# samiazirar/mvtracker

Hardware: AMD Instinct MI355X
Metric: query-points*frames/sec, 4-view 24-frame 512x512 @1024 queries (higher is better)
Workload: dtype bf16; 1 GPU; c3: 4-view synthetic 24-frame 512x512, 1024 queries, bf16 (configs[2], the metric's config); 4-view 24-frame 512x512, 1024 queries per GPU, corr K=16 x 4 levels, iters=4, 3 windows, random-init weights (seeded recipe); queries_total=1024, parallelism=query-shard x1, frame_store=bf16 rows

## Files before the change

include/mvtracker_hip.h:

```cpp
#ifndef MVTRACKER_HIP_H
#define MVTRACKER_HIP_H

#include <stdint.h>

#ifdef __cplusplus
extern "C" {
#endif

#define MVT_OK 0
#define MVT_ERR_ARG 1
#define MVT_ERR_HIP_BASE 1000

#define MVT_ACT_NONE 0
#define MVT_ACT_RELU 1
#define MVT_ACT_GELU_TANH 2
#define MVT_ACT_GELU_ERF 3

int mvt_abi_version(void);
const char* mvt_build_arch(void);

int mvt_gemm(const float* A, int lda, const float* Wt, int ldw, const float* bias, const float* R, int ldr,
             float* C, int ldc, int M, int N, int K, int act, void* stream);

int mvt_conv2d(const float* in, const float* wt, const float* bias, float* out, int n, int H, int W, int Cin,
// ... 2 lines not shown
int mvt_split_bf16(const float* src, unsigned short* hi, unsigned short* lo, long long n, void* stream);
int mvt_gemm_bf16(const float* A, int lda, const unsigned short* w_hi, const unsigned short* w_lo, int ldw,
                  const float* bias, const float* R, int ldr, void* C, int ldc, int M, int N, int K, int act,
                  int io_flags , void* stream);
#define MVT_IO_IN_BF16 1
#define MVT_IO_OUT_BF16 2
#define MVT_IO_SHORT_WG 4
int mvt_conv2d_stat_slots(int H, int W, int Cin, int KH, int KW, int stride, int pad, int split );
int mvt_conv3x3s2_down_bf16(const void* in, const unsigned short* w3, const float* b3, const unsigned short* wd, const float* bd,
                            void* out3, void* outd, int n, int H, int W, int Cin, int Cout, int ldo, float* part3, float* partd,
                            void* stream);
int mvt_conv2d_bf16(const void* in, const unsigned short* wt_hi, const unsigned short* wt_lo, const float* bias,
                    void* out, int n, int H, int W, int Cin, int Cout, int KH, int KW, int stride, int pad, int ldo,
                    int act, int io_flags, const float* in_stats, float* out_partial, void* stream);
int mvt_instnorm_finish_slots(const float* partial, int slots, float* mean_rstd, int n, long long HW, int C, void* stream);

int mvt_ln_gemm_bf16(const float* A, int lda, const float* ln_w, const float* ln_b, float ln_eps,
                     const unsigned short* w_hi, const unsigned short* w_lo, int ldw, const float* bias, const float* R,
                     int ldr, float* C, int ldc, int M, int N, int K, int act, void* stream);

int mvt_mlp_fused_bf16(float* x, int ldx, const unsigned short* w1, int ldw1, const float* b1,
                       const unsigned short* w2, int ldw2, const float* b2, long long M, int C, int H, float eps,
                       void* stream);

int mvt_pack_frag_bf16(const unsigned short* w, int ld, int N, int K, unsigned short* out, void* stream);
typedef struct mvt_block_next {
  const unsigned short* w;
  const float* b;
  const float* lnw;
  const float* lnb;
// ... 389 lines not shown
```

mvtracker_amd/csrc/conv_rows.hip:

```cpp
#include <stdlib.h>

#include "common.h"

namespace {

typedef __bf16 bf16x8 __attribute__((ext_vector_type(8)));
typedef __bf16 bf16x4 __attribute__((ext_vector_type(4)));
typedef unsigned u32x4 __attribute__((ext_vector_type(4)));
typedef unsigned u32x2 __attribute__((ext_vector_type(2)));
typedef float f32x2 __attribute__((ext_vector_type(2)));
typedef short s16x2 __attribute__((ext_vector_type(2)));
typedef __bf16 bf16x2 __attribute__((ext_vector_type(2)));

#ifdef MVT_STAMPS
#ifndef MVT_STAMP_WG
#define MVT_STAMP_WG 2000
#endif
__device__ unsigned long long mvt_conv_stamp_buf[2 * 8 * 128];
#define CSTAMP(i)                                                                                                  \
  do {                                                                                                             \
    __builtin_amdgcn_sched_barrier(0);                                                                             \
    unsigned long long t_;                                                                                         \
    asm volatile("s_memtime %0\n\ts_waitcnt lgkmcnt(0)" : "=s"(t_)::"memory");                                     \
    __builtin_amdgcn_sched_barrier(0);                                                                             \
// ... 918 lines not shown
}
#endif

static int rows_nw8() {
  static const int v = getenv("MVT_ROWS_NW8") ? atoi(getenv("MVT_ROWS_NW8")) : 0;
  return v;
}
__attribute__((visibility("hidden"))) int mvt_detail_conv_rows_tile_rows(int ksize, int stride, int Ho) {
  if (ksize == 3 && stride == 1) return (rows_nw8() == 1 && Ho % 16 == 0) ? 16 : (rows_nw8() == 2 ? 4 : 8);
  if (ksize == 3) return 4;
  if (ksize == 7) return TR;
  return 8;
}
__attribute__((visibility("hidden"))) int mvt_detail_conv_rows_slots(int Ho, int Wo, int tile_rows) {
  return (int)(mvt_cdiv(Ho, tile_rows) * mvt_cdiv(Wo, TC));
}

__attribute__((visibility("hidden"))) int mvt_detail_conv_rows(const void* in, const unsigned short* w, int ldw, const float* bias, void* out,
                                                               int n, int H, int W, int Cin, int Cout, int ksize, int stride, int ldo,
                                                               int io_flags, const float* in_stats, float* out_partial,
                                                               hipStream_t stream) {
  MVT_REQUIRE((ksize == 1 || ksize == 3) && (stride == 1 || stride == 2));
  MVT_REQUIRE((!in_stats || Cin <= MAXC) && Cin % CK == 0 && (long long)H * W * Cin < (1LL << 31) && (long long)Cout * ldw < (1LL << 31));
  MVT_REQUIRE((long long)(TC + 8) * ldo * 4 < (1LL << 31));
  const int pad = ksize == 3 ? 1 : 0;
  const int Ho = (H + 2 * pad - ksize) / stride + 1, Wo = (W + 2 * pad - ksize) / stride + 1;
  RowsArgs a{};
  a.in = (const float*)in; a.w = w; a.bias = bias; a.out = (float*)out; a.in_stats = in_stats; a.out_part = out_partial;
  a.H = H; a.W = W; a.Cin = Cin; a.Cout = Cout; a.ldw = ldw; a.ldo = ldo;
  a.slots = mvt_detail_conv_rows_slots(Ho, Wo, mvt_detail_conv_rows_tile_rows(ksize, stride, Ho));
// ... 13 lines not shown
    const long long tiles = (long long)n * mvt_cdiv(Ho, NW_ * TM_) * mvt_cdiv(Wo, TC) * mvt_cdiv(Cout, bn);                        \
    MVT_REQUIRE(tiles < (1LL << 31));                                                                                              \
    const dim3 grid((unsigned)tiles);                                                                                              \
    if (n96) {                                                                                                                     \
      if (a.in_bf16) LAUNCH2(TM_, 3, KS_, S_, NW_, true);                                                                          \
      else LAUNCH2(TM_, 3, KS_, S_, NW_, false);                                                                                   \
    } else {                                                                                                                       \
      if (a.in_bf16) LAUNCH2(TM_, 2, KS_, S_, NW_, true);                                                                          \
      else LAUNCH2(TM_, 2, KS_, S_, NW_, false);                                                                                   \
    }                                                                                                                              \
  } while (0)
  const int nw8 = rows_nw8();
  if (ksize == 3 && stride == 1 && !in_stats && !(io_flags & MVT_IO_SHORT_WG) && a.in_bf16 && st_ok && Cout % BG_BN == 0 && ((uintptr_t)in & 15) == 0 && Cin % 8 == 0 &&
      ldw % 8 == 0 && ((uintptr_t)w & 15) == 0 && (long long)Cout * ldw * 2 < (1LL << 31) && (long long)H * W * Cin * 2 < (1LL << 31)) {
    const char* e = getenv("MVT_CONV_BIG");
    if (!e || atoi(e) != 0) {
      const long long tiles = (long long)n * mvt_cdiv(Ho, TR) * mvt_cdiv(Wo, TC) * (Cout / BG_BN);
      MVT_REQUIRE(tiles < (1LL << 31));
      hipLaunchKernelGGL(conv3x3_big_bf16, dim3((unsigned)tiles), dim3(512), 0, stream, a);
      return mvt_launch_status();
    }
  }
  if (ksize == 3 && stride == 1 && nw8 == 1 && Ho % 16 == 0) LAUNCH(2, 3, 1, 8);
  else if (ksize == 3 && stride == 1 && nw8 == 2) LAUNCH(1, 3, 1, 4);
  else if (ksize == 3 && stride == 1) LAUNCH(2, 3, 1, 4);
  else if (ksize == 3) LAUNCH(1, 3, 2, 4);
  else if (stride == 1) LAUNCH(2, 1, 1, 4);
  else LAUNCH(2, 1, 2, 4);
#undef LAUNCH2
#undef LAUNCH
  return mvt_launch_status();
}
// ... 62 lines not shown
```

mvtracker_amd/csrc/encoder.hip:

```cpp
#include <stdlib.h>

#include "common.h"

namespace {

template <typename TIN>
__global__ void rgb_to_nhwc4_kernel(const TIN* __restrict__ rgbs, float* __restrict__ out, int V, int T, int H, int W,
                                    long long img0, long long nimg) {
  const long long hw = (long long)H * W;
  const long long total = nimg * hw;
  for (long long i = blockIdx.x * (long long)blockDim.x + threadIdx.x; i < total; i += (long long)gridDim.x * blockDim.x) {
    long long img = i / hw;
    long long pix = i - img * hw;
    int tt = (int)((img0 + img) / V), v = (int)((img0 + img) - (long long)tt * V);
    const TIN* src = rgbs + (((long long)v * T + tt) * 3) * hw + pix;
    f32x4 o;
    o[0] = 2.0f * ((float)src[0] / 255.0f) - 1.0f;
    o[1] = 2.0f * ((float)src[hw] / 255.0f) - 1.0f;
    o[2] = 2.0f * ((float)src[2 * hw] / 255.0f) - 1.0f;
    o[3] = 0.0f;
    *reinterpret_cast<f32x4*>(out + i * 4) = o;
  }
}

// ... 65 lines not shown
  double s = 0, ss = 0;
  for (int slab = 0; slab < MVT_IN_SLABS; ++slab) {
    const double* p = partial + ((img * MVT_IN_SLABS + slab) * C + c) * 2;
    s += p[0];
    ss += p[1];
  }
  double mean = s / (double)HW;
  double var = ss / (double)HW - mean * mean;
  if (var < 0) var = 0;
  mean_rstd[i * 2] = (float)mean;
  mean_rstd[i * 2 + 1] = (float)(1.0 / sqrt(var + 1e-5));
}

constexpr int FC = 8, FL = 1024 / FC;
__global__ __launch_bounds__(1024) void instnorm_finish_slots_kernel(const float* __restrict__ partial, int slots,
                                                                     float* __restrict__ mean_rstd, long long HW, int C) {
  __shared__ double red[1024 * 2];
  const int t = threadIdx.x, c = blockIdx.x * FC + (t % FC), l = t / FC;
  const long long img = blockIdx.y;
  double s = 0, ss = 0;
  if (c < C) {
    for (int sl = l; sl < slots; sl += FL) {
      const float2 v = *reinterpret_cast<const float2*>(partial + ((img * slots + sl) * C + c) * 2);
      s += (double)v.x;
      ss += (double)v.y;
    }
  }
  red[t * 2] = s;
  red[t * 2 + 1] = ss;
  __syncthreads();
  for (int w = FL / 2; w >= 1; w >>= 1) {
    if (l < w) {
      red[t * 2] += red[(t + w * FC) * 2];
      red[t * 2 + 1] += red[(t + w * FC) * 2 + 1];
// ... 326 lines not shown
                                  int io_flags, void* stream) {
  MVT_REQUIRE((io_flags & ~MVT_IO_IN_BF16) == 0);
  MVT_REQUIRE(x && partial && mean_rstd && n > 0 && HW > 0 && C > 0 && C % 4 == 0 && C <= 256 && ldx >= C && ldx % 4 == 0);
  MVT_REQUIRE(256 % (C / 4) == 0 || C / 4 <= 64);
  hipLaunchKernelGGL(instnorm_partial_kernel, dim3(MVT_IN_SLABS, n), dim3(256), 0, mvt_stream(stream), (const float*)x, ldx, partial,
                     HW, C, io_flags & MVT_IO_IN_BF16 ? 1 : 0);
  long long total = (long long)n * C;
  hipLaunchKernelGGL(instnorm_finish_kernel, dim3((unsigned)mvt_cdiv(total, 256)), dim3(256), 0, mvt_stream(stream), partial,
                     mean_rstd, HW, C, total);
  return mvt_launch_status();
}

extern "C" int mvt_instnorm_finish_slots(const float* partial, int slots, float* mean_rstd, int n, long long HW, int C, void* stream) {
  MVT_REQUIRE(partial && mean_rstd && slots > 0 && n > 0 && HW > 0 && C > 0);
  hipLaunchKernelGGL(instnorm_finish_slots_kernel, dim3((unsigned)mvt_cdiv(C, FC), (unsigned)n), dim3(1024), 0, mvt_stream(stream),
                     partial, slots, mean_rstd, HW, C);
  return mvt_launch_status();
}

extern "C" int mvt_instnorm_apply(const void* x, const float* mean_rstd, const void* skip, const float* skip_stats, void* y,
                                  int n, long long HW, int C, int io_flags, void* stream) {
  MVT_REQUIRE(x && mean_rstd && y && n > 0 && HW > 0 && C > 0 && C % 4 == 0);
  const int both = MVT_IO_IN_BF16 | MVT_IO_OUT_BF16;
  const int skip_relu = io_flags & MVT_APPLY_SKIP_RELU ? 1 : 0;
  io_flags &= ~MVT_APPLY_SKIP_RELU;
  MVT_REQUIRE(io_flags == 0 || io_flags == both);
  MVT_REQUIRE(!skip_relu || skip_stats);
  MVT_REQUIRE(skip || !skip_stats);
  static const bool generic = getenv("MVT_APPLY_GENERIC") != nullptr;
  if (io_flags && C % 8 == 0 && C <= 2048 && HW < (1LL << 31) && !generic && ((uintptr_t)x % 16 == 0) && ((uintptr_t)y % 16 == 0) &&
      ((uintptr_t)skip % 16 == 0)) {
// ... 34 lines not shown
```

mvtracker_amd/csrc/encoder_forward.hip:

```cpp
#include "common.h"
#include <stdlib.h>

namespace {

inline long long align256(long long b) { return (b + 255) & ~255LL; }

struct Plan {
  long long stem, z0, y, s[4], d, cat, c2, part, st, total;
  long long st_ch;
};

inline Plan plan(long long n, int H, int W, int C) {
  const long long h2 = H / 2, w2 = W / 2, hs = H / 4, ws = W / 4;
  Plan P{};
  long long o = 0;
  auto take = [&](long long bytes) { const long long at = o; o += align256(bytes); return at; };
  const long long big = n * h2 * w2 * 64 * 2;
  P.stem = take(big);
  P.z0 = take(big);
  P.y = take(big);
  const int couts[4] = {64, 96, 128, 128};
  long long hh = h2, ww = w2;
  for (int l = 0; l < 4; ++l) {
    if (l) {
// ... 6 lines not shown
  P.cat = take(n * hs * ws * 416 * 2);
  P.c2 = take(n * hs * ws * 2 * C * 2);
  const long long slots_max = ((h2 + 7) / 8) * ((w2 + 31) / 32);
  P.st_ch = 2 * C > 256 ? 2 * C : 256;
  P.part = take(n * slots_max * P.st_ch * 2 * 4);
  P.st = take(8 * n * P.st_ch * 2 * 4);
  P.total = o;
  return P;
}

constexpr long long GROUP_BUDGET_SHARED = 80LL << 20;
inline int group_size(int n, int h2, int w2, int shared, int* g_out) {
  long long g = shared ? GROUP_BUDGET_SHARED / (3LL * h2 * w2 * 64 * 2) : n;
  if (g < 1) g = n;
  if (const char* e = getenv("MVT_ENC_GROUP")) {
    const long v = strtol(e, nullptr, 10);
    if (v < 0) return MVT_ERR_ARG;
    if (v > 0) g = v;
  }
  *g_out = (int)(g > n ? n : g);
  return MVT_OK;
}

}

extern "C" long long mvt_encoder_workspace_bytes(int n, int H, int W, int C) {
  if (n <= 0 || H < 16 || W < 16 || C <= 0) return -1;
  return plan(n, H, W, C).total;
}

// ... 34 lines not shown

  auto conv = [&](int ci, const void* in, int io_in, void* out, int hh, int ww, int cin, int cout, int k, int stride, int pad, int ld_out,
                  const float* in_stats, float** st_out, int io_out) -> int {
    const mvt_conv_weights& cw = w->conv[ci];
    const int ho = (hh + 2 * pad - k) / stride + 1, wo = (ww + 2 * pad - k) / stride + 1;
    const long long in_img = (long long)hh * ww * cin * (io_in & MVT_IO_IN_BF16 ? 2 : 4);
    const long long out_img = (long long)ho * wo * ld_out * (io_out & MVT_IO_OUT_BF16 ? 2 : 4);
    float* pp = nullptr;
    int slots = 0;
    if (st_out) {
      slots = mvt_conv2d_stat_slots(hh, ww, cin, k, k, stride, pad, 0);
      MVT_REQUIRE(slots > 0);
      pp = part + (long long)ga * slots * cout * 2;
    }
    ENC_TRY(mvt_conv2d_bf16(img(in, in_img), cw.w, nullptr, cw.b, img(out, out_img), gn, hh, ww, cin, cout, k, k, stride, pad, ld_out,
                            MVT_ACT_NONE, io_in | io_out | (w->short_workgroups ? MVT_IO_SHORT_WG : 0), rows_of(in_stats, cin), pp, stream));
    if (st_out) {
      *st_out = new_st();
      ENC_TRY(mvt_instnorm_finish_slots(pp, slots, (float*)rows_of(*st_out, cout), gn, (long long)ho * wo, cout, stream));
    }
    return MVT_OK;
  };

  auto stem = [&](float** st_stem) -> int {
    if (x4) return conv(0, x4, 0, base + P.stem, H, W, 4, 64, 7, 2, 3, 64, nullptr, st_stem, MVT_IO_OUT_BF16);
    const mvt_conv_weights& cw = w->conv[0];
    const int slots = mvt_detail_conv_rows_slots(h2, w2, mvt_detail_conv_rows_tile_rows(7, 2, h2));
    float* pp = part + (long long)ga * slots * 64 * 2;
    ENC_TRY(mvt_detail_stem7x7_rows_src(nullptr, rgb, rgb_u8, rgb_V, rgb_T, img0 + ga, cw.w, (7 * 32 + 63) & ~63, cw.b,
                                        img(base + P.stem, (long long)h2 * w2 * 64 * 2), gn, H, W, 64, 64, MVT_IO_OUT_BF16, pp, mvt_stream(stream)));
    *st_stem = new_st();
// ... 3 lines not shown
  auto res_block = [&](int c1, int c2, int cd, const void* xin, const float* x_stats, int hh, int ww, int cin, int cout, int stride,
                       void* zout) -> int {
    const int ho = (hh + 2 - 3) / stride + 1, wo = (ww + 2 - 3) / stride + 1;
    const long long in_img = (long long)hh * ww * cin * 2, out_img = (long long)ho * wo * cout * 2;
    float *s1 = nullptr, *s2 = nullptr, *sd = nullptr;
    static const bool no_fold = getenv("MVT_FOLD_DOWNSAMPLE") && atoi(getenv("MVT_FOLD_DOWNSAMPLE")) == 0;
    const bool fold = cd >= 0 && stride == 2 && !x_stats && cout % 32 == 0 && !no_fold;
    if (fold) {
      const int slots = mvt_conv2d_stat_slots(hh, ww, cin, 3, 3, 2, 1, 0);
      MVT_REQUIRE(slots > 0);
      float* part_3 = part + (long long)ga * slots * cout * 2;
      float* part_d = part_3 + (long long)n * slots * cout * 2;
      ENC_TRY(mvt_conv3x3s2_down_bf16(img(xin, in_img), w->conv[c1].w, w->conv[c1].b, w->conv[cd].w, w->conv[cd].b, img(base + P.y, out_img),
                                      img(base + P.d, out_img), gn, hh, ww, cin, cout, cout, part_3, part_d, stream));
      s1 = new_st();
      ENC_TRY(mvt_instnorm_finish_slots(part_3, slots, (float*)rows_of(s1, cout), gn, (long long)ho * wo, cout, stream));
      sd = new_st();
      ENC_TRY(mvt_instnorm_finish_slots(part_d, slots, (float*)rows_of(sd, cout), gn, (long long)ho * wo, cout, stream));
    } else {
      ENC_TRY(conv(c1, xin, MVT_IO_IN_BF16, base + P.y, hh, ww, cin, cout, 3, stride, 1, cout, x_stats, &s1, MVT_IO_OUT_BF16));
    }
    ENC_TRY(conv(c2, base + P.y, MVT_IO_IN_BF16, zout, ho, wo, cout, cout, 3, 1, 1, cout, s1, &s2, MVT_IO_OUT_BF16));
    const void* skip = xin;
    long long skip_img = in_img;
    const float* skip_stats = x_stats;
    int flags = BF | (x_stats ? MVT_APPLY_SKIP_RELU : 0);
    if (cd >= 0) {
      if (!fold) ENC_TRY(conv(cd, xin, MVT_IO_IN_BF16, base + P.d, hh, ww, cin, cout, 1, stride, 0, cout, nullptr, &sd, MVT_IO_OUT_BF16));
      skip = base + P.d;
      skip_img = out_img;
      skip_stats = sd;
      flags = BF;
    }
// ... 13 lines not shown
  for (ga = 0; ga < n; ga += g) {
    gn = n - ga < g ? n - ga : g;
    st_next = 0;
    float* st_stem = nullptr;
    ENC_TRY(stem(&st_stem));
    ENC_TRY(layer(0, base + P.stem, st_stem, h2, w2, 64));
  }
  ga = 0, gn = n;
  const void* stage[4] = {base + P.s[0]};
  int sh[4] = {h2}, sw[4] = {w2}, sc[4] = {64};
  for (int l = 1; l < 4; ++l) {
    ENC_TRY(layer(l, base + P.s[l - 1], nullptr, sh[l - 1], sw[l - 1], sc[l - 1]));
    stage[l] = base + P.s[l]; sh[l] = (sh[l - 1] - 1) / 2 + 1; sw[l] = (sw[l - 1] - 1) / 2 + 1; sc[l] = couts[l];
  }
  const int hs = H / 4, ws = W / 4;
  ENC_TRY(mvt_concat_resize_bilinear_ac(4, stage, sh, sw, sc, base + P.cat, n, hs, ws, 416, BF, stream));
  float* st_c2 = nullptr;
  ENC_TRY(conv(21, base + P.cat, MVT_IO_IN_BF16, base + P.c2, hs, ws, 416, 2 * C, 3, 1, 1, 2 * C, nullptr, &st_c2, MVT_IO_OUT_BF16));
  ENC_TRY(conv(22, base + P.c2, MVT_IO_IN_BF16, out_rows, hs, ws, 2 * C, C, 1, 1, 0, ldo, st_c2, nullptr, out_bf16 ? MVT_IO_OUT_BF16 : 0));
  return MVT_OK;
}

extern "C" int mvt_encoder_forward(const mvt_encoder_weights* w, const float* x4, int n, int H, int W, void* out_rows, int ldo,
                                   int out_bf16, void* workspace, long long workspace_bytes, void* stream) {
  MVT_REQUIRE(x4);
  return encoder_run(w, x4, nullptr, 0, 0, 0, 0, n, H, W, out_rows, ldo, out_bf16, workspace, workspace_bytes, stream);
}

extern "C" int mvt_encoder_forward_rgb(const mvt_encoder_weights* w, const void* rgbs, int is_u8, int V, int T, long long img0, int n, int H,
                                       int W, void* out_rows, int ldo, int out_bf16, void* workspace, long long workspace_bytes,
                                       void* stream) {
  MVT_REQUIRE(rgbs && (is_u8 == 0 || is_u8 == 1) && V > 0 && T > 0 && img0 >= 0 && n > 0 && img0 + n <= (long long)V * T);
  return encoder_run(w, nullptr, rgbs, is_u8, V, T, img0, n, H, W, out_rows, ldo, out_bf16, workspace, workspace_bytes, stream);
}
// ... 1 lines not shown
```

mvtracker_amd/hip.py:

```python
from __future__ import annotations

import contextlib
import ctypes as C
import functools
import os

import torch

_HERE = os.path.dirname(os.path.abspath(__file__))
LIB_PATH = os.environ.get("MVT_LIB") or os.path.join(_HERE, "lib", "libmvtracker_hip.so")

if not os.path.exists(LIB_PATH):
    raise RuntimeError(
        f"{LIB_PATH} not found: the HIP library is required (no fallback path exists). "
        "Build it with `python -m mvtracker_amd.build`.")
_lib = C.CDLL(LIB_PATH)

P, I, LL, F = C.c_void_p, C.c_int, C.c_longlong, C.c_float

SIGNATURES = {
    "mvt_abi_version": [],
    "mvt_build_arch": [],
    "mvt_gemm": [P, I, P, I, P, P, I, P, I, I, I, I, I, P],
    "mvt_conv2d": [P, P, P, P, I, I, I, I, I, I, I, I, I, I, I, P],
    "mvt_split_bf16": [P, P, P, LL, P],
    "mvt_gemm_bf16": [P, I, P, P, I, P, P, I, P, I, I, I, I, I, I, P],
    "mvt_conv2d_stat_slots": [I, I, I, I, I, I, I, I],
    "mvt_conv2d_bf16": [P, P, P, P, P, I, I, I, I, I, I, I, I, I, I, I, I, P, P, P],
    "mvt_conv3x3s2_down_bf16": [P, P, P, P, P, P, P, I, I, I, I, I, I, P, P, P],
    "mvt_instnorm_finish_slots": [P, I, P, I, LL, I, P],
    "mvt_ln_gemm_bf16": [P, I, P, P, F, P, P, I, P, P, I, P, I, I, I, I, I, P],
    "mvt_pack_frag_bf16": [P, I, I, I, P, P],
    "mvt_block_fused_bf16": [P, I, P, I, I, I, P, I, P, P, I, P, P, I, P, I, P, I, LL, I, P, P],
    "mvt_mlp_fused_bf16": [P, I, P, I, P, P, I, P, LL, I, I, F, P],
    "mvt_rgb_to_nhwc4": [P, P, I, I, I, I, I, I, P],
    "mvt_rgb_u8_to_nhwc4": [P, P, I, I, I, I, I, I, P],
    "mvt_rgb_images_to_nhwc4": [P, I, P, I, I, I, I, LL, I, P],
    "mvt_resize_nearest": [P, P, LL, I, I, I, I, P],
    "mvt_instnorm_stats": [P, I, P, P, I, LL, I, I, P],
    "mvt_instnorm_apply": [P, P, P, P, P, I, LL, I, I, P],
    "mvt_resize_bilinear_ac": [P, P, I, I, I, I, I, I, I, I, I, P],
    "mvt_concat_resize_bilinear_ac": [I, P, P, P, P, P, I, I, I, I, I, P],
    "mvt_invert_cameras": [P, P, P, P, I, P],
    "mvt_depth_subsample": [P, P, I, I, I, I, I, P],
    "mvt_avgpool2": [P, P, LL, I, I, I, I, P],
# ... 187 lines not shown
                out_partial=None, short_wg=False):
    _call("mvt_conv2d_bf16", _ptr(x), _ptr(wt_hi), _ptr(wt_lo), _ptr(bias), _ptr(out), n, H, W, Cin, Cout, KH, KW, stride, pad,
          ldo, act, _io(x, out) | (IO_SHORT_WG if short_wg else 0), _ptr(in_stats), _ptr(out_partial), _stream())


def conv3x3s2_down_bf16(x, w3, b3, wd, bd, out3, outd, n, H, W, Cin, Cout, ldo, part3=None, partd=None):
    assert x.dtype == torch.bfloat16 and out3.dtype == torch.bfloat16 and outd.dtype == torch.bfloat16
    _call("mvt_conv3x3s2_down_bf16", _ptr(x), _ptr(w3), _ptr(b3), _ptr(wd), _ptr(bd), _ptr(out3), _ptr(outd), n, H, W, Cin, Cout, ldo,
          _ptr(part3), _ptr(partd), _stream())


def instnorm_finish_slots(partial, slots, mean_rstd, n, HW, Cc):
    _call("mvt_instnorm_finish_slots", _ptr(partial), slots, _ptr(mean_rstd), n, HW, Cc, _stream())


def ln_gemm_bf16(A, lda, ln_w, ln_b, eps, Whi, Wlo, ldw, bias, R, ldr, Cm, ldc, M, N, K, act=ACT_NONE):
    _call("mvt_ln_gemm_bf16", _ptr(A), lda, _ptr(ln_w), _ptr(ln_b), eps, _ptr(Whi), _ptr(Wlo), ldw, _ptr(bias), _ptr(R), ldr,
          _ptr(Cm), ldc, M, N, K, act, _stream())


def pack_frag_bf16(w, ld, N, K, out):
    _call("mvt_pack_frag_bf16", _ptr(w), ld, N, K, _ptr(out), _stream())


class BlockNext(C.Structure):
    _fields_ = [("w", C.c_void_p), ("b", C.c_void_p), ("lnw", C.c_void_p), ("lnb", C.c_void_p), ("y", C.c_void_p),
                ("ldw", C.c_int), ("N", C.c_int), ("ldy", C.c_int), ("eps", C.c_float), ("row_lo", C.c_longlong),
                ("row_hi", C.c_longlong), ("y_bf16", C.c_int)]


# ... 765 lines not shown
```

mvtracker_amd/parallel.py:

```python
from __future__ import annotations

import logging
import os
from typing import Optional

import torch
import torch.distributed as dist

from . import hip

log = logging.getLogger(__name__)


class ShardedTracker:
    def __init__(self, model, group: Optional["dist.ProcessGroup"] = None):
        self.model = model
        self.group = group
        self.staged = os.environ.get("MVT_GATHER_INPLACE", "0") == "0"
        self.last_store = None

    def open_stream(self, *args, **kwargs):
        raise NotImplementedError("there is no streaming form of ShardedTracker (a ring frame store sharded over ranks is not built): "
                                  "open the session on one rank's model, MVTracker.open_stream")

# ... 64 lines not shown
                if hi > lo:
                    m.encode_images(r0, base + lo, base + hi, storage)
                if hi - lo < per:
                    storage[base + rank * per + (hi - lo):base + (rank + 1) * per].zero_()
                self._all_gather_in_place(dst, rank, world)

            first_end = min(T, t0 + m.S)
            two_blocks = m.overlap_encoder and first_end < T
            exchange_block(t0, first_end if two_blocks else T)
            store = m.build_frame_store(r0, d0, i0, e0, t0=t0, level0=level0, t1=first_end if two_blocks else T)
            if two_blocks and dev.type == "cuda":
                main = torch.cuda.current_stream(dev)
                side = m._side_stream(dev)
                side.wait_stream(main)
                with torch.cuda.stream(side):
                    with m._beside_windows(short_workgroups=m.wide_conv_shared != "1"):
                        exchange_block(first_end, T)
                    m.fill_frame_features(store, r0, first_end, T, level0=level0)
                    ev = torch.cuda.Event()
                    ev.record(side)
                store["pending"] = [(first_end, ev)]
                for t_ in (r0, storage):
                    t_.record_stream(side)
            elif two_blocks:
                exchange_block(first_end, T)
                m.fill_frame_features(store, r0, first_end, T, level0=level0)
        self.last_store = store
        res = m(rgbs, depths, query_points[:, a:b], intrs, extrs, iters=iters, frame_store=store, **opts)
        if not gather_output:
            return res
        per = (N + world - 1) // world
# ... 20 lines not shown
```

mvtracker_amd/tracker.py:

```python
from __future__ import annotations

import contextlib
import logging
import math
import os
from typing import Dict, Optional, Tuple

import numpy as np
import torch
from torch import nn

from . import hip
from .backward import reversed_layout, window_prefixes
from .grouped import grouped_layout

log = logging.getLogger(__name__)


_param_epoch = [0]


class _Node(nn.Module):

    def register_parameter(self, name, param):
# ... 103 lines not shown
        self.fuse_blocks = True
        self.mfma_attention = True
        self.overlap_encoder = os.environ.get("MVT_OVERLAP", "1") != "0"
        self._side = {}
        self._scratch = {}
        self.bf16_tokens = os.environ.get("MVT_BF16_TOK", "1") != "0"
        self.bf16_activations = os.environ.get("MVT_BF16_ACT", "1") != "0"
        self.bf16_store = os.environ.get("MVT_BF16_STORE", "1") != "0"
        self.fuse_attention = int(os.environ.get("MVT_FUSE_ATTN", "55"))
        self.seed_across_windows = os.environ.get("MVT_SEED_WINDOWS", "1") != "0"
        self.encoder_chunk_images = int(os.environ.get("MVT_ENC_CHUNK", "0"))
        self.encoder_streams = int(os.environ.get("MVT_ENC_STREAMS", "2"))
        self.presearch = os.environ.get("MVT_PRESEARCH", "1") != "0"
        self.stem_reads_clip = os.environ.get("MVT_STEM_RGB", "1") != "0"
        self.wide_conv_shared = os.environ.get("MVT_CONV_BIG_SHARED", "auto")
        self._shared_gpu = False
        self.sync_debug = os.environ.get("MVT_SYNC_DEBUG", "0") != "0"
        self.composite_encoder = os.environ.get("MVT_COMPOSITE_ENCODER", "1") != "0"
        self.fuse_tokens = os.environ.get("MVT_FUSE_TOKENS", "1") != "0"
        self.fuse_input = os.environ.get("MVT_FUSE_INPUT", "1") != "0"
        self.fuse_head = os.environ.get("MVT_FUSE_HEAD", "1") != "0"
        self.fuse_norm = True
        self.fold_downsample = os.environ.get("MVT_FOLD_DOWNSAMPLE", "1") != "0"
        d = self.updateformer_input_dim
        self._time_embed_host = self._make_time_embed(self.S, d)

    def _shapes(self) -> Dict[str, Tuple[int, ...]]:
        s: Dict[str, Tuple[int, ...]] = {}

        def wb(name, *shape):
            s[name + ".weight"] = tuple(shape)
# ... 142 lines not shown
                for nme in (".cross_attn.to_q", ".cross_attn.to_kv", ".cross_attn.to_out", ".mlp.fc1", ".mlp.fc2"):
                    lin(p + nme)
        pk["virtual"] = sd[u + "virual_tracks"].reshape(self.nv, self.hidden).contiguous()
        if self._composite_updater_ok():
            pk["updater_struct"] = self._updater_struct(pk, sd, matrix)
        if self._composite_encoder_ok():
            ew = hip.EncoderWeights()
            ew.latent_dim = self.latent_dim
            names = ["fnet.conv1"]
            for li in range(1, 5):
                names += [f"fnet.layer{li}.0.conv1", f"fnet.layer{li}.0.conv2", f"fnet.layer{li}.0.downsample.0" if li > 1 else f"fnet.layer{li}.0.conv1",
                          f"fnet.layer{li}.1.conv1", f"fnet.layer{li}.1.conv2"]
            names += ["fnet.conv2", "fnet.conv3"]
            ews = hip.EncoderWeights()
            ews.latent_dim, ews.short_workgroups = self.latent_dim, 1
            for i, nm in enumerate(names):
                ew.conv[i].w, ew.conv[i].b = pk[nm][0][0].data_ptr(), pk[nm][1].data_ptr()
                ews.conv[i].w, ews.conv[i].b = ew.conv[i].w, ew.conv[i].b
            pk["encoder_struct"], pk["encoder_struct_shared"] = ew, ews
        pk["ffeats_norm"] = (sd["ffeats_norm.weight"].contiguous(), sd["ffeats_norm.bias"].contiguous())
        lin("ffeats_updater.0")
        pk["vis"] = (sd["vis_predictor.0.weight"].reshape(-1).contiguous(), sd["vis_predictor.0.bias"].contiguous())
        pk["time_embed"] = self._time_embed_host.to(dev)
        a3 = _round_up(self.updateformer_input_dim, 6) // 3
        om = np.arange(a3 // 2, dtype=np.float64)
        om /= a3 / 2.0
        pk["pos_omega"] = torch.from_numpy(1.0 / 10000 ** om).to(dev)
        self._packed, self._packed_sig = pk, sig
        return pk

    def _composite_updater_ok(self):
        return (self.precision == "bf16" and self.hidden == 256 and self.num_heads == 6 and self.dim_head == 48 and self.nv == 64
                and self.latent_dim == 128 and self.fuse_blocks and self.mfma_attention and self.bf16_tokens
                and self.depth <= hip.UPDATER_MAX_DEPTH and hip.COMPOSITE and os.environ.get("MVT_COMPOSITE", "1") != "0")
# ... 65 lines not shown
        pk["updater_struct_keep"] = keep
        return w

    def _conv(self, pk, name, x, n, H, W, cin, cout, k, stride, pad, out=None, ldo=None, in_stats=None, stats=False):
        wt, b = pk[name]
        Ho = (H + 2 * pad - k) // stride + 1
        Wo = (W + 2 * pad - k) // stride + 1
        if out is None:
            out = torch.empty(n, Ho, Wo, cout, device=x.device, dtype=self._act_dtype(pk))
            ldo = cout
        st = None
        if isinstance(wt, tuple):
            slots = hip.conv2d_stat_slots(H, W, cin, k, k, stride, pad, wt[1] is not None) if (stats and self.fuse_norm) else 0
            part = torch.empty(n * slots * cout * 2, device=x.device) if slots else None
            hip.conv2d_bf16(x, wt[0], wt[1], b, out, n, H, W, cin, cout, k, k, stride, pad, ldo, in_stats=in_stats, out_partial=part,
                            short_wg=self._shared_gpu)
            if slots:
                st = torch.empty(n, cout, 2, device=x.device)
                hip.instnorm_finish_slots(part, slots, st, n, Ho * Wo, cout)
        else:
            assert in_stats is None
            hip.conv2d(x, wt, b, out, n, H, W, cin, cout, k, k, stride, pad, ldo)
        if stats and st is None:
            st = self._inorm(out, n, Ho * Wo, cout, apply=False)
        return (out, Ho, Wo, st) if stats else (out, Ho, Wo)

    def store_dtype(self):
        return torch.bfloat16 if (self.precision == "bf16" and self.bf16_store) else torch.float32

    def _act_dtype(self, pk):
        return torch.bfloat16 if (self.bf16_activations and self.precision == "bf16") else torch.float32
# ... 29 lines not shown
        if not fuse_in:
            self._inorm(y, n, Ho * Wo, cout, st=st1)
        y2, _, _, st2 = self._conv(pk, p + ".conv2", y, n, Ho, Wo, cout, cout, 3, 1, 1, in_stats=st1 if fuse_in else None,
                                   stats=True)
        if (p + ".downsample.0") in pk:
            if d is None:
                d, _, _, dst = self._conv(pk, p + ".downsample.0", x, n, H, W, cin, cout, 1, stride, 0, stats=True)
            self._inorm(y2, n, Ho * Wo, cout, skip=d, skip_stats=dst, st=st2)
        else:
            self._inorm(y2, n, Ho * Wo, cout, skip=x, skip_stats=x_stats, skip_relu=x_stats is not None, st=st2)
        return y2, Ho, Wo

    def _encode(self, pk, x4, n, H, W, out_rows):
        C = self.latent_dim
        composite = "encoder_struct" in pk and out_rows.is_contiguous()
        est = "encoder_struct_shared" if self._shared_gpu else "encoder_struct"
        if isinstance(x4, _ClipImages):
            src = x4
            if composite and self.stem_reads_clip:
                ws = self._workspace(hip.encoder_workspace_bytes(n, H, W, C), src.rgbs.device)
                return hip.encoder_forward_rgb(pk[est], src.rgbs, src.V, src.T, src.img0, n, H, W, out_rows, C, ws)
            x4 = torch.empty(n, H, W, 4, device=src.rgbs.device)
            hip.rgb_images_to_nhwc4(src.rgbs, x4, src.V, src.T, H, W, src.img0, n)
        if composite:
            ws = self._workspace(hip.encoder_workspace_bytes(n, H, W, C), x4.device)
            return hip.encoder_forward(pk[est], x4, n, H, W, out_rows, C, ws)
        hs, ws = H // self.stride, W // self.stride
        x, h, w, st = self._conv(pk, "fnet.conv1", x4, n, H, W, 4, 64, 7, 2, 3, stats=True)
        lazy_stem = self.fuse_norm and self.precision == "bf16"
        if not lazy_stem:
            self._inorm(x, n, h * w, 64, st=st)
# ... 85 lines not shown
            torch.cuda.synchronize(dev)

    def _helper_stream(self, dev):
        key = ("helper", dev.type, dev.index)
        if key not in self._side:
            self._side[key] = torch.cuda.Stream(device=dev)
        return self._side[key]

    def _side_stream(self, dev):
        key = (dev.type, dev.index)
        if key not in self._side:
            self._side[key] = torch.cuda.Stream(device=dev)
        return self._side[key]

    @contextlib.contextmanager
    def _beside_windows(self, short_workgroups=True):
        self._shared_gpu = short_workgroups
        try:
            yield
        finally:
            self._shared_gpu = False

    def _encode_on_side_stream(self, store, rgbs, firsts, pending, end=None):
        dev = rgbs.device
        S = self.S
        T = rgbs.shape[1] if end is None else min(end, rgbs.shape[1])
        streams = [self._side_stream(dev)]
        for st in streams:
            st.wait_stream(torch.cuda.current_stream(dev))
        self._handover(dev)
        V = rgbs.shape[0]
        first_block = max(1, min(rgbs.shape[1], S)) * V
        side_images = sum(min(T, a + S // 2) - a for a in firsts) * V
        big = self.wide_conv_shared == "1" or (self.wide_conv_shared == "auto" and side_images > 2 * first_block)
        for i, a in enumerate(firsts):
            st = streams[i % len(streams)]
            with torch.cuda.stream(st):
                with self._beside_windows(short_workgroups=not big):
                    self.fill_frame_features(store, rgbs, a, min(T, a + S // 2))
                ev = torch.cuda.Event()
                ev.record(st)
                pending.append((a, ev))

    @hip.guarded
    def fill_frame_features(self, store, rgbs, a, b, level0=None, after_first_chunk=None):
        V, T, _, H, W = rgbs.shape
        hs, ws = H // self.stride, W // self.stride
        fv = store["fvec"]
        if level0 is None:
            self.encode_frames(rgbs, a, b, images_per_chunk=self.encoder_chunk_images or max(16, V * (self.S // 2)), out=fv[0],
                               after_first_chunk=after_first_chunk)
        elif after_first_chunk is not None:
            after_first_chunk()
# ... 744 lines not shown
```

Measured before the change: 1.054 million query-points*frames/s.

## Add side-stream encoder mode with grouped tail convs and batched norm finish

```diff
diff --git a/include/mvtracker_hip.h b/include/mvtracker_hip.h
--- a/include/mvtracker_hip.h
+++ b/include/mvtracker_hip.h
@@ -40,6 +40,8 @@
                     void* out, int n, int H, int W, int Cin, int Cout, int KH, int KW, int stride, int pad, int ldo,
                     int act, int io_flags, const float* in_stats, float* out_partial, void* stream);
 int mvt_instnorm_finish_slots(const float* partial, int slots, float* mean_rstd, int n, long long HW, int C, void* stream);
+int mvt_instnorm_finish_slots_tables(const float* partial, long long partial_stride, int slots, float* mean_rstd, long long table_stride,
+                                     int tables, int n, long long HW, int C, void* stream);
 
 int mvt_ln_gemm_bf16(const float* A, int lda, const float* ln_w, const float* ln_b, float ln_eps,
                      const unsigned short* w_hi, const unsigned short* w_lo, int ldw, const float* bias, const float* R,
diff --git a/mvtracker_amd/csrc/conv_rows.hip b/mvtracker_amd/csrc/conv_rows.hip
--- a/mvtracker_amd/csrc/conv_rows.hip
+++ b/mvtracker_amd/csrc/conv_rows.hip
@@ -956,6 +956,10 @@
 }
 __attribute__((visibility("hidden"))) int mvt_detail_conv_rows_slots(int Ho, int Wo, int tile_rows) {
   return (int)(mvt_cdiv(Ho, tile_rows) * mvt_cdiv(Wo, TC));
+}
+
+__attribute__((visibility("hidden"))) long long mvt_detail_conv_big_tiles(int Ho, int Wo, int Cout) {
+  return mvt_cdiv(Ho, TR) * mvt_cdiv(Wo, TC) * (Cout / BG_BN);
 }
 
 __attribute__((visibility("hidden"))) int mvt_detail_conv_rows(const void* in, const unsigned short* w, int ldw, const float* bias, void* out,
@@ -999,8 +1003,10 @@
   if (ksize == 3 && stride == 1 && !in_stats && !(io_flags & MVT_IO_SHORT_WG) && a.in_bf16 && st_ok && Cout % BG_BN == 0 && ((uintptr_t)in & 15) == 0 && Cin % 8 == 0 &&
       ldw % 8 == 0 && ((uintptr_t)w & 15) == 0 && (long long)Cout * ldw * 2 < (1LL << 31) && (long long)H * W * Cin * 2 < (1LL << 31)) {
     const char* e = getenv("MVT_CONV_BIG");
-    if (!e || atoi(e) != 0) {
-      const long long tiles = (long long)n * mvt_cdiv(Ho, TR) * mvt_cdiv(Wo, TC) * (Cout / BG_BN);
+    const int big_slots = mvt_detail_conv_rows_slots(Ho, Wo, TR);
+    if ((!e || atoi(e) != 0) && (!out_partial || big_slots == a.slots)) {
+      a.slots = big_slots;
+      const long long tiles = n * mvt_detail_conv_big_tiles(Ho, Wo, Cout);
       MVT_REQUIRE(tiles < (1LL << 31));
       hipLaunchKernelGGL(conv3x3_big_bf16, dim3((unsigned)tiles), dim3(512), 0, stream, a);
       return mvt_launch_status();
diff --git a/mvtracker_amd/csrc/encoder.hip b/mvtracker_amd/csrc/encoder.hip
--- a/mvtracker_amd/csrc/encoder.hip
+++ b/mvtracker_amd/csrc/encoder.hip
@@ -103,10 +103,13 @@
 
 constexpr int FC = 8, FL = 1024 / FC;
 __global__ __launch_bounds__(1024) void instnorm_finish_slots_kernel(const float* __restrict__ partial, int slots,
-                                                                     float* __restrict__ mean_rstd, long long HW, int C) {
+                                                                     float* __restrict__ mean_rstd, long long HW, int C,
+                                                                     long long partial_stride, long long table_stride) {
   __shared__ double red[1024 * 2];
   const int t = threadIdx.x, c = blockIdx.x * FC + (t % FC), l = t / FC;
   const long long img = blockIdx.y;
+  partial += blockIdx.z * partial_stride;
+  mean_rstd += blockIdx.z * table_stride;
   double s = 0, ss = 0;
   if (c < C) {
     for (int sl = l; sl < slots; sl += FL) {
@@ -463,7 +466,16 @@
 extern "C" int mvt_instnorm_finish_slots(const float* partial, int slots, float* mean_rstd, int n, long long HW, int C, void* stream) {
   MVT_REQUIRE(partial && mean_rstd && slots > 0 && n > 0 && HW > 0 && C > 0);
   hipLaunchKernelGGL(instnorm_finish_slots_kernel, dim3((unsigned)mvt_cdiv(C, FC), (unsigned)n), dim3(1024), 0, mvt_stream(stream),
-                     partial, slots, mean_rstd, HW, C);
+                     partial, slots, mean_rstd, HW, C, 0LL, 0LL);
+  return mvt_launch_status();
+}
+
+extern "C" int mvt_instnorm_finish_slots_tables(const float* partial, long long partial_stride, int slots, float* mean_rstd,
+                                                long long table_stride, int tables, int n, long long HW, int C, void* stream) {
+  MVT_REQUIRE(partial && mean_rstd && slots > 0 && n > 0 && n <= 65535 && HW > 0 && C > 0 && tables > 0 && tables <= 65535);
+  MVT_REQUIRE(partial_stride % 2 == 0);
+  hipLaunchKernelGGL(instnorm_finish_slots_kernel, dim3((unsigned)mvt_cdiv(C, FC), (unsigned)n, (unsigned)tables), dim3(1024), 0,
+                     mvt_stream(stream), partial, slots, mean_rstd, HW, C, partial_stride, table_stride);
   return mvt_launch_status();
 }
 
diff --git a/mvtracker_amd/csrc/encoder_forward.hip b/mvtracker_amd/csrc/encoder_forward.hip
--- a/mvtracker_amd/csrc/encoder_forward.hip
+++ b/mvtracker_amd/csrc/encoder_forward.hip
@@ -1,5 +1,7 @@
 #include "common.h"
 #include <stdlib.h>
+
+long long mvt_detail_conv_big_tiles(int Ho, int Wo, int Cout);
 
 namespace {
 
@@ -44,6 +46,34 @@
   long long g = shared ? GROUP_BUDGET_SHARED / (3LL * h2 * w2 * 64 * 2) : n;
   if (g < 1) g = n;
   if (const char* e = getenv("MVT_ENC_GROUP")) {
+    const long v = strtol(e, nullptr, 10);
+    if (v < 0) return MVT_ERR_ARG;
+    if (v > 0) g = v;
+  }
+  *g_out = (int)(g > n ? n : g);
+  return MVT_OK;
+}
+
+inline int cu_count() {
+  static int cus[64];
+  int dev = 0;
+  if (hipGetDevice(&dev) != hipSuccess || dev < 0 || dev >= 64) return 0;
+  if (!cus[dev]) {
+    int v = 0;
+    if (hipDeviceGetAttribute(&v, hipDeviceAttributeMultiprocessorCount, dev) != hipSuccess) return 0;
+    cus[dev] = v;
+  }
+  return cus[dev];
+}
+
+inline int tail_group_size(int n, int hs, int ws, int cout, int mode, int* g_out) {
+  long long g = n;
+  if (mode & 2) {
+    const long long tiles = mvt_detail_conv_big_tiles(hs, ws, cout);
+    g = 2LL * cu_count() / (tiles > 0 ? tiles : 1);
+    if (g < 1) g = n;
+  }
+  if (const char* e = getenv("MVT_ENC_TAIL_GROUP")) {
     const long v = strtol(e, nullptr, 10);
     if (v < 0) return MVT_ERR_ARG;
     if (v > 0) g = v;
@@ -108,7 +138,7 @@
       pp = part + (long long)ga * slots * cout * 2;
     }
     ENC_TRY(mvt_conv2d_bf16(img(in, in_img), cw.w, nullptr, cw.b, img(out, out_img), gn, hh, ww, cin, cout, k, k, stride, pad, ld_out,
-                            MVT_ACT_NONE, io_in | io_out | (w->short_workgroups ? MVT_IO_SHORT_WG : 0), rows_of(in_stats, cin), pp, stream));
+                            MVT_ACT_NONE, io_in | io_out | (w->short_workgroups & 1 ? MVT_IO_SHORT_WG : 0), rows_of(in_stats, cin), pp, stream));
     if (st_out) {
       *st_out = new_st();
       ENC_TRY(mvt_instnorm_finish_slots(pp, slots, (float*)rows_of(*st_out, cout), gn, (long long)ho * wo, cout, stream));
@@ -142,9 +172,9 @@
       ENC_TRY(mvt_conv3x3s2_down_bf16(img(xin, in_img), w->conv[c1].w, w->conv[c1].b, w->conv[cd].w, w->conv[cd].b, img(base + P.y, out_img),
                                       img(base + P.d, out_img), gn, hh, ww, cin, cout, cout, part_3, part_d, stream));
       s1 = new_st();
-      ENC_TRY(mvt_instnorm_finish_slots(part_3, slots, (float*)rows_of(s1, cout), gn, (long long)ho * wo, cout, stream));
       sd = new_st();
-      ENC_TRY(mvt_instnorm_finish_slots(part_d, slots, (float*)rows_of(sd, cout), gn, (long long)ho * wo, cout, stream));
+      ENC_TRY(mvt_instnorm_finish_slots_tables(part_3, part_d - part_3, slots, (float*)rows_of(s1, cout), sd - s1, 2, gn, (long long)ho * wo,
+                                               cout, stream));
     } else {
       ENC_TRY(conv(c1, xin, MVT_IO_IN_BF16, base + P.y, hh, ww, cin, cout, 3, stride, 1, cout, x_stats, &s1, MVT_IO_OUT_BF16));
     }
@@ -188,10 +218,19 @@
     stage[l] = base + P.s[l]; sh[l] = (sh[l - 1] - 1) / 2 + 1; sw[l] = (sw[l - 1] - 1) / 2 + 1; sc[l] = couts[l];
   }
   const int hs = H / 4, ws = W / 4;
-  ENC_TRY(mvt_concat_resize_bilinear_ac(4, stage, sh, sw, sc, base + P.cat, n, hs, ws, 416, BF, stream));
-  float* st_c2 = nullptr;
-  ENC_TRY(conv(21, base + P.cat, MVT_IO_IN_BF16, base + P.c2, hs, ws, 416, 2 * C, 3, 1, 1, 2 * C, nullptr, &st_c2, MVT_IO_OUT_BF16));
-  ENC_TRY(conv(22, base + P.c2, MVT_IO_IN_BF16, out_rows, hs, ws, 2 * C, C, 1, 1, 0, ldo, st_c2, nullptr, out_bf16 ? MVT_IO_OUT_BF16 : 0));
+  int gt = n;
+  ENC_TRY(tail_group_size(n, hs, ws, 2 * C, w->short_workgroups, &gt));
+  const int st_tail = st_next;
+  for (ga = 0; ga < n; ga += gt) {
+    gn = n - ga < gt ? n - ga : gt;
+    st_next = st_tail;
+    const void* src[4];
+    for (int l = 0; l < 4; ++l) src[l] = img(stage[l], (long long)sh[l] * sw[l] * sc[l] * 2);
+    ENC_TRY(mvt_concat_resize_bilinear_ac(4, src, sh, sw, sc, img(base + P.cat, (long long)hs * ws * 416 * 2), gn, hs, ws, 416, BF, stream));
+    float* st_c2 = nullptr;
+    ENC_TRY(conv(21, base + P.cat, MVT_IO_IN_BF16, base + P.c2, hs, ws, 416, 2 * C, 3, 1, 1, 2 * C, nullptr, &st_c2, MVT_IO_OUT_BF16));
+    ENC_TRY(conv(22, base + P.c2, MVT_IO_IN_BF16, out_rows, hs, ws, 2 * C, C, 1, 1, 0, ldo, st_c2, nullptr, out_bf16 ? MVT_IO_OUT_BF16 : 0));
+  }
   return MVT_OK;
 }
 
diff --git a/mvtracker_amd/hip.py b/mvtracker_amd/hip.py
--- a/mvtracker_amd/hip.py
+++ b/mvtracker_amd/hip.py
@@ -29,6 +29,7 @@
     "mvt_conv2d_bf16": [P, P, P, P, P, I, I, I, I, I, I, I, I, I, I, I, I, P, P, P],
     "mvt_conv3x3s2_down_bf16": [P, P, P, P, P, P, P, I, I, I, I, I, I, P, P, P],
     "mvt_instnorm_finish_slots": [P, I, P, I, LL, I, P],
+    "mvt_instnorm_finish_slots_tables": [P, LL, I, P, LL, I, I, LL, I, P],
     "mvt_ln_gemm_bf16": [P, I, P, P, F, P, P, I, P, P, I, P, I, I, I, I, I, P],
     "mvt_pack_frag_bf16": [P, I, I, I, P, P],
     "mvt_block_fused_bf16": [P, I, P, I, I, I, P, I, P, P, I, P, P, I, P, I, P, I, LL, I, P, P],
@@ -246,6 +247,13 @@
     _call("mvt_instnorm_finish_slots", _ptr(partial), slots, _ptr(mean_rstd), n, HW, Cc, _stream())
 
 
+def instnorm_finish_slots_tables(partial, slots, mean_rstd, n, HW, Cc):
+    tables = mean_rstd.shape[0]
+    assert partial.shape[0] == tables and partial.is_contiguous() and mean_rstd.is_contiguous()
+    _call("mvt_instnorm_finish_slots_tables", _ptr(partial), partial.stride(0), slots, _ptr(mean_rstd), mean_rstd.stride(0), tables, n,
+          HW, Cc, _stream())
+
+
 def ln_gemm_bf16(A, lda, ln_w, ln_b, eps, Whi, Wlo, ldw, bias, R, ldr, Cm, ldc, M, N, K, act=ACT_NONE):
     _call("mvt_ln_gemm_bf16", _ptr(A), lda, _ptr(ln_w), _ptr(ln_b), eps, _ptr(Whi), _ptr(Wlo), ldw, _ptr(bias), _ptr(R), ldr,
           _ptr(Cm), ldc, M, N, K, act, _stream())
diff --git a/mvtracker_amd/parallel.py b/mvtracker_amd/parallel.py
--- a/mvtracker_amd/parallel.py
+++ b/mvtracker_amd/parallel.py
@@ -102,7 +102,7 @@
                 side = m._side_stream(dev)
                 side.wait_stream(main)
                 with torch.cuda.stream(side):
-                    with m._beside_windows(short_workgroups=m.wide_conv_shared != "1"):
+                    with m._beside_windows(m.side_encoder_mode((T - first_end) * V, (first_end - t0) * V)):
                         exchange_block(first_end, T)
                     m.fill_frame_features(store, r0, first_end, T, level0=level0)
                     ev = torch.cuda.Event()
diff --git a/mvtracker_amd/tracker.py b/mvtracker_amd/tracker.py
--- a/mvtracker_amd/tracker.py
+++ b/mvtracker_amd/tracker.py
@@ -141,7 +141,7 @@
         self.presearch = os.environ.get("MVT_PRESEARCH", "1") != "0"
         self.stem_reads_clip = os.environ.get("MVT_STEM_RGB", "1") != "0"
         self.wide_conv_shared = os.environ.get("MVT_CONV_BIG_SHARED", "auto")
-        self._shared_gpu = False
+        self._shared_gpu = 0
         self.sync_debug = os.environ.get("MVT_SYNC_DEBUG", "0") != "0"
         self.composite_encoder = os.environ.get("MVT_COMPOSITE_ENCODER", "1") != "0"
         self.fuse_tokens = os.environ.get("MVT_FUSE_TOKENS", "1") != "0"
@@ -314,10 +314,13 @@
             names += ["fnet.conv2", "fnet.conv3"]
             ews = hip.EncoderWeights()
             ews.latent_dim, ews.short_workgroups = self.latent_dim, 1
+            ewl = hip.EncoderWeights()
+            ewl.latent_dim, ewl.short_workgroups = self.latent_dim, 2
             for i, nm in enumerate(names):
                 ew.conv[i].w, ew.conv[i].b = pk[nm][0][0].data_ptr(), pk[nm][1].data_ptr()
                 ews.conv[i].w, ews.conv[i].b = ew.conv[i].w, ew.conv[i].b
-            pk["encoder_struct"], pk["encoder_struct_shared"] = ew, ews
+                ewl.conv[i].w, ewl.conv[i].b = ew.conv[i].w, ew.conv[i].b
+            pk["encoder_struct"], pk["encoder_struct_shared"], pk["encoder_struct_launches"] = ew, ews, ewl
         pk["ffeats_norm"] = (sd["ffeats_norm.weight"].contiguous(), sd["ffeats_norm.bias"].contiguous())
         lin("ffeats_updater.0")
         pk["vis"] = (sd["vis_predictor.0.weight"].reshape(-1).contiguous(), sd["vis_predictor.0.bias"].contiguous())
@@ -413,7 +416,7 @@
             slots = hip.conv2d_stat_slots(H, W, cin, k, k, stride, pad, wt[1] is not None) if (stats and self.fuse_norm) else 0
             part = torch.empty(n * slots * cout * 2, device=x.device) if slots else None
             hip.conv2d_bf16(x, wt[0], wt[1], b, out, n, H, W, cin, cout, k, k, stride, pad, ldo, in_stats=in_stats, out_partial=part,
-                            short_wg=self._shared_gpu)
+                            short_wg=bool(self._shared_gpu & 1))
             if slots:
                 st = torch.empty(n, cout, 2, device=x.device)
                 hip.instnorm_finish_slots(part, slots, st, n, Ho * Wo, cout)
@@ -473,7 +476,7 @@
     def _encode(self, pk, x4, n, H, W, out_rows):
         C = self.latent_dim
         composite = "encoder_struct" in pk and out_rows.is_contiguous()
-        est = "encoder_struct_shared" if self._shared_gpu else "encoder_struct"
+        est = ("encoder_struct", "encoder_struct_shared", "encoder_struct_launches")[self._shared_gpu]
         if isinstance(x4, _ClipImages):
             src = x4
             if composite and self.stem_reads_clip:
@@ -589,12 +592,17 @@
         return self._side[key]
 
     @contextlib.contextmanager
-    def _beside_windows(self, short_workgroups=True):
-        self._shared_gpu = short_workgroups
+    def _beside_windows(self, mode=1):
+        self._shared_gpu = mode
         try:
             yield
         finally:
-            self._shared_gpu = False
+            self._shared_gpu = 0
+
+    def side_encoder_mode(self, side_images, first_block_images):
+        if self.wide_conv_shared in ("0", "1", "2"):
+            return {"0": 1, "1": 0, "2": 2}[self.wide_conv_shared]
+        return 0 if side_images > 2 * first_block_images else 2
 
     def _encode_on_side_stream(self, store, rgbs, firsts, pending, end=None):
         dev = rgbs.device
@@ -607,11 +615,11 @@
         V = rgbs.shape[0]
         first_block = max(1, min(rgbs.shape[1], S)) * V
         side_images = sum(min(T, a + S // 2) - a for a in firsts) * V
-        big = self.wide_conv_shared == "1" or (self.wide_conv_shared == "auto" and side_images > 2 * first_block)
+        mode = self.side_encoder_mode(side_images, first_block)
         for i, a in enumerate(firsts):
             st = streams[i % len(streams)]
             with torch.cuda.stream(st):
-                with self._beside_windows(short_workgroups=not big):
+                with self._beside_windows(mode):
                     self.fill_frame_features(store, rgbs, a, min(T, a + S // 2))
                 ev = torch.cuda.Event()
                 ev.record(st)
```

Result: no change. 1.062 million query-points*frames/s, median of 6 (+0.8%).
